# SamuelGong/FLASHE

Hardware: AMD Instinct MI355X
Metric: ciphertexts/sec (enc+agg+dec), 1e7-elem vector; achieved HBM GB/s fraction (higher is better)
Workload: dtype u128

## Files before the change

### flashe_amd/csrc/abi.hip

```cpp
#include "ctx.h"
#include "blockpool.h"

#include <algorithm>
#include <cstdarg>
#include <cstdio>
#include <cstdlib>
#include <cmath>
#include <cstring>
#include <mutex>
#include <new>
#include <string>
#include <vector>

using namespace flashe;

namespace {

struct AesTables {
    uint8_t sbox[256];
    uint32_t te0[256];
    AesTables()
    {
        uint8_t alog[256], lg[256];
        uint8_t x = 1;
// ... 761 lines not shown
        if (rc) return rc;
    }
    if (ctx->env.prf_backend != PRF_AUTO && ctx->env.prf_backend != PRF_TABLE) {
        for (int v = 0; v < n_vec; v++) {
            int rc = flashe_encrypt_dev(ctx, iter, idx[v], scheme, n, n_jobs, pt_dev[v], pt_limbs, ct_dev[v]);
            if (rc) return rc;
        }
        return FLASHE_OK;
    }
    return batch_shares(ctx, n_vec, [&](int v0, int nv) {
        return launch_prf_batch(ctx->env, iter, scheme == FLASHE_SCHEME_DOUBLE, nv, idx + v0, pt_dev + v0, pt_limbs, ct_dev + v0, n, n_jobs);
    });
}

static int check_range(flashe_ctx *ctx, uint64_t n, uint64_t first, uint64_t count);
static int check_u32(flashe_ctx *ctx, uint64_t n, uint32_t n_jobs)
{
    if (ctx->int_bits > 32) return fail(ctx, FLASHE_EINVAL, "the uint32 layout needs int_bits <= 32, this ctx has %d", ctx->int_bits);
    if (n >= (1ull << 32)) return fail(ctx, FLASHE_EINVAL, "the uint32 layout needs n < 2^32");
    if (n_jobs == 0) return fail(ctx, FLASHE_EINVAL, "n_jobs must be >= 1");
    if (ctx->env.prf_backend != PRF_AUTO && ctx->env.prf_backend != PRF_TABLE) return fail(ctx, FLASHE_EINVAL, "the uint32 layout runs on the table PRF only");
    if (!ctx->env.use_chain) return fail(ctx, FLASHE_EINVAL, "the uint32 layout needs the chained kernels (FLASHE_CHAIN=0 is set)");
    return FLASHE_OK;
}

int flashe_encrypt_batch_u32_dev(flashe_ctx *ctx, uint32_t iter, int scheme, uint64_t n, uint32_t n_jobs, int n_vec, const uint32_t *idx,
                                 const uint32_t *const *pt_dev, uint32_t *const *ct_dev)
{
    CHECK_CTX(ctx);
    if (int rc = check_scheme(ctx, scheme)) return rc;
// ... 21 lines not shown
    if (reinterpret_cast<uintptr_t>(sum_out_dev) & 3u) return fail(ctx, FLASHE_EINVAL, "sum_out_dev must be 4-byte aligned");
    if (n && ct_dev) { if (int rc = check_sum_apart(ctx, sum_out_dev, n_vec, pt_dev, ct_dev)) return rc; }
    if (scheme == FLASHE_SCHEME_DOUBLE && n && n_vec > 0 && n_vec <= kMaxUniformBatch && idx && pt_dev && ct_dev) {
        int rc = check_u32(ctx, n, n_jobs);
        if (rc || (rc = check_double_idx(ctx, scheme, idx, n_vec))) return rc;
        bool ok = true;
        for (int v = 0; v < n_vec && ok; v++)
            ok = pt_dev[v] && ct_dev[v] && !((reinterpret_cast<uintptr_t>(pt_dev[v]) | reinterpret_cast<uintptr_t>(ct_dev[v])) & 3u) && (v == 0 || idx[v] == idx[v - 1] + 1u);
        if (ok) {
            LaunchEnv env = ctx->env;
            env.elem32 = 1;
            std::vector<uint32_t> sidx(idx, idx + n_vec);
            sidx.push_back(idx[n_vec - 1] + 1u);
            PrfChain ch{sidx.data(), n_vec, false, 0, n, reinterpret_cast<const uint64_t *const *>(pt_dev), 1, reinterpret_cast<uint64_t *const *>(ct_dev)};
            ch.sum_out_dev = reinterpret_cast<uint64_t *>(sum_out_dev);
            const hipError_t e = launch_prf_chains(env, iter, 1, &ch, n, n_jobs);
            if (e == hipSuccess) return FLASHE_OK;
            if (e != hipErrorNotSupported) HIP_TRY(ctx, e);
        }
    }
    int rc = flashe_encrypt_batch_u32_dev(ctx, iter, scheme, n, n_jobs, n_vec, idx, pt_dev, ct_dev);
    if (rc || n == 0) return rc;
    if (n_vec == 0) { HIP_TRY(ctx, hipMemsetAsync(sum_out_dev, 0, n * 4, ctx->env.stream)); return FLASHE_OK; }
    return flashe_aggregate_elem_u32_dev(ctx, n_vec, ct_dev, n, sum_out_dev);
}

int flashe_aggregate_decrypt_u32_dev(flashe_ctx *ctx, uint32_t iter, const uint32_t *add_idx, int n_add, const uint32_t *minus_idx, int n_minus,
                                     uint64_t n, uint32_t n_jobs, uint64_t first, uint64_t count, int C, const uint32_t *const *cts_dev,
                                     void *agg_out_dev, void *out_dev, int out_elem_bytes)
{
    CHECK_CTX(ctx);
    if (C < 1 || C > kMaxOps || !cts_dev || (count && !out_dev)) return fail(ctx, FLASHE_EINVAL, "aggregate_decrypt_u32: bad arguments (C = %d, at most %d)", C, kMaxOps);
    if (out_elem_bytes != 4 && out_elem_bytes != 8) return fail(ctx, FLASHE_EINVAL, "out_elem_bytes must be 4 or 8");
    if (n_add != 1 || n_minus < 0 || n_minus > 1 || !add_idx || (n_minus && !minus_idx))
        return fail(ctx, FLASHE_EINVAL, "aggregate_decrypt_u32: one add and at most one minus prefix (widen the vectors for prefix lists)");
    int rc = check_u32(ctx, n, n_jobs);
    if (rc) return rc;
    rc = check_range(ctx, n, first, count);
    if (rc) return rc;
    if (count == 0) return FLASHE_OK;
    if ((rc = check_operands(ctx, C, cts_dev, 4))) return rc;
    const uintptr_t need = static_cast<uintptr_t>(out_elem_bytes - 1);
    if ((reinterpret_cast<uintptr_t>(out_dev) | reinterpret_cast<uintptr_t>(agg_out_dev)) & need) return fail(ctx, FLASHE_EINVAL, "outputs must be %d-byte aligned", out_elem_bytes);
    LaunchEnv env = ctx->env;
    env.elem32 = 1;
    if (C == 1 && !agg_out_dev && out_elem_bytes == 4 && n_minus == 1) {
        const uint32_t sidx[2] = {add_idx[0], minus_idx[0]};
        const uint64_t *in1 = reinterpret_cast<const uint64_t *>(cts_dev[0]);
        uint64_t *out1 = static_cast<uint64_t *>(out_dev);
        PrfChain ch{sidx, 1, false, first, count, &in1, 1, &out1};
        const hipError_t e = launch_prf_chains(env, iter, 1, &ch, n, n_jobs);
        if (e == hipSuccess) return FLASHE_OK;
        if (e != hipErrorNotSupported) HIP_TRY(ctx, e);
    }
    HIP_TRY(ctx, launch_small_reduce_decrypt(env, iter, add_idx[0], n_minus == 1, n_minus ? minus_idx[0] : 0u, n, n_jobs, first, count, C,
                                             reinterpret_cast<const uint64_t *const *>(cts_dev), static_cast<uint64_t *>(agg_out_dev),
                                             static_cast<uint64_t *>(out_dev), out_elem_bytes));
    return FLASHE_OK;
}

int flashe_aggregate_elem_u32_dev(flashe_ctx *ctx, int C, const uint32_t *const *cts_dev, uint64_t n, uint32_t *out_dev)
// ... 19 lines not shown
{
    CHECK_CTX(ctx);
    if (n && (!in_dev || !out_dev)) return fail(ctx, FLASHE_EINVAL, "widen_u32: null vector");
    HIP_TRY(ctx, launch_widen_u32(ctx->env, n, in_dev, out_dev));
    return FLASHE_OK;
}

int flashe_narrow_u32_dev(flashe_ctx *ctx, uint64_t n, const uint64_t *in_dev, uint32_t *out_dev)
{
    CHECK_CTX(ctx);
    if (n && (!in_dev || !out_dev)) return fail(ctx, FLASHE_EINVAL, "narrow_u32: null vector");
    HIP_TRY(ctx, launch_narrow_u32(ctx->env, n, in_dev, out_dev));
    return FLASHE_OK;
}

static uint64_t *chain_dmask_begin(flashe_ctx *ctx, uint64_t count)
{
    flashe_ctx::ChainDmask &s = ctx->chain_dmask;
    s.valid = false;
    if (!ctx->chain_dmask_on || ctx->capturing || ctx->limbs != 2 || count == 0) return nullptr;
    if (ensure(ctx, s.d, vec_bytes(ctx, count)) != FLASHE_OK) {
        (void)hipGetLastError();
        ctx->err.clear();
        return nullptr;
    }
    return static_cast<uint64_t *>(s.d.p);
}

static void chain_dmask_commit(flashe_ctx *ctx, uint32_t iter, const uint32_t *idx, int n_vec, uint64_t n, uint32_t n_jobs, uint64_t first,
                               uint64_t count)
{
    flashe_ctx::ChainDmask &s = ctx->chain_dmask;
    s.iter = iter; s.key_epoch = ctx->key_epoch; s.add_idx = idx[n_vec - 1] + 1u; s.minus_idx = idx[0];
    s.n = n; s.n_jobs = n_jobs; s.first = first; s.count = count;
    s.valid = true;
}

static const uint64_t *chain_dmask_match(const flashe_ctx *ctx, uint32_t iter, const uint32_t *add_idx, int n_add, const uint32_t *minus_idx,
                                         int n_minus, uint64_t n, uint32_t n_jobs, uint64_t first, uint64_t count)
{
    const flashe_ctx::ChainDmask &s = ctx->chain_dmask;
    if (!s.valid || ctx->capturing || n_add != 1 || n_minus != 1 || count == 0) return nullptr;
    if (add_idx[0] != s.add_idx || minus_idx[0] != s.minus_idx || iter != s.iter || ctx->key_epoch != s.key_epoch || n != s.n ||
        n_jobs != s.n_jobs)
        return nullptr;
    if (first < s.first || first - s.first > s.count || count > s.count - (first - s.first)) return nullptr;
    return static_cast<const uint64_t *>(s.d.p) + (first - s.first) * 2;
}

int flashe_encrypt_batch_sum_dev(flashe_ctx *ctx, uint32_t iter, int scheme, uint64_t n, uint32_t n_jobs, int n_vec, const uint32_t *idx,
                                 const uint64_t *const *pt_dev, int pt_limbs, uint64_t *const *ct_dev, uint64_t *sum_out_dev)
{
    CHECK_CTX(ctx);
    if (!sum_out_dev && n && n_vec) return fail(ctx, FLASHE_EINVAL, "flashe_encrypt_batch_sum_dev: null sum_out_dev");
    if (n_vec > 0) { if (int rc = check_double_idx(ctx, scheme, idx, n_vec)) return rc; }
    if (n && n_vec) {
        if (int rc = check_sum_aligned(ctx, sum_out_dev)) return rc;
        if (int rc = check_sum_apart(ctx, sum_out_dev, n_vec, pt_dev, ct_dev)) return rc;
    }
    if (scheme == FLASHE_SCHEME_DOUBLE && n && n_vec > 0 && idx && pt_dev && ct_dev) {
        bool ok = true;
        for (int v = 0; v < n_vec && ok; v++) ok = pt_dev[v] && ct_dev[v];
        if (ok) {
            for (int v = 0; v < n_vec; v++) {
                int rc = check_prf_args(ctx, 1, scheme, n_jobs, ct_dev[v], pt_dev[v], pt_limbs);
                if (rc) return rc;
            }
            uint64_t *const dmask = chain_dmask_begin(ctx, n);
            const hipError_t e = launch_prf_batch_sum(ctx->env, iter, n_vec, idx, pt_dev, pt_limbs, ct_dev, sum_out_dev, n, n_jobs, 0, n, dmask);
            if (e == hipSuccess) {
                if (dmask) chain_dmask_commit(ctx, iter, idx, n_vec, n, n_jobs, 0, n);
                return FLASHE_OK;
            }
            if (e != hipErrorNotSupported) HIP_TRY(ctx, e);
        }
    }
    int rc = flashe_encrypt_batch_dev(ctx, iter, scheme, n, n_jobs, n_vec, idx, pt_dev, pt_limbs, ct_dev);
    if (rc || n == 0) return rc;
    if (n_vec == 0) { HIP_TRY(ctx, hipMemsetAsync(sum_out_dev, 0, n * ctx->limbs * 8, ctx->env.stream)); return FLASHE_OK; }
    return flashe_aggregate_elem_dev(ctx, n_vec, ct_dev, n, sum_out_dev);
}

int flashe_prf_jobs_dev(flashe_ctx *ctx, uint32_t iter, uint64_t n, uint32_t n_jobs, int n_entries, const flashe_prf_job *entries)
{
    CHECK_CTX(ctx);
    if (n_entries < 0 || (n_entries && !entries)) return fail(ctx, FLASHE_EINVAL, "bad job list");
// ... 813 lines not shown
    int rc = check_range(ctx, n, first, count);
    if (rc || (rc = check_double_idx(ctx, scheme, idx, n_vec))) return rc;
    if (n_jobs == 0) return fail(ctx, FLASHE_EINVAL, "n_jobs must be >= 1");
    if (ctx->env.prf_backend != PRF_AUTO && ctx->env.prf_backend != PRF_TABLE) return fail(ctx, FLASHE_EINVAL, "encrypt_batch_range runs on the table PRF only");
    for (int v = 0; v < n_vec; v++) {
        if (count && (!pt_dev[v] || !ct_dev[v])) return fail(ctx, FLASHE_EINVAL, "null vector %d", v);
        if (sum_out_dev && (ct_dev[v] == sum_out_dev || pt_dev[v] == sum_out_dev))
            return fail(ctx, FLASHE_EINVAL, "sum_out_dev must not be one of the plaintext or ciphertext vectors");
        rc = check_prf_args(ctx, 1, scheme, n_jobs, ct_dev[v], pt_dev[v], pt_limbs);
        if (rc) return rc;
    }
    if (sum_out_dev && (rc = check_sum_aligned(ctx, sum_out_dev))) return rc;
    if (count == 0) return FLASHE_OK;
    if (n_vec == 0) { if (sum_out_dev) HIP_TRY(ctx, hipMemsetAsync(sum_out_dev, 0, vec_bytes(ctx, count), ctx->env.stream)); return FLASHE_OK; }
    if (sum_out_dev && scheme == FLASHE_SCHEME_DOUBLE) {
        uint64_t *const dmask = chain_dmask_begin(ctx, count);
        const hipError_t e = launch_prf_batch_sum(ctx->env, iter, n_vec, idx, pt_dev, pt_limbs, ct_dev, sum_out_dev, n, n_jobs, first, count, dmask);
        if (e == hipSuccess) {
            if (dmask) chain_dmask_commit(ctx, iter, idx, n_vec, n, n_jobs, first, count);
            return FLASHE_OK;
        }
        if (e != hipErrorNotSupported) HIP_TRY(ctx, e);
    }
    rc = batch_shares(ctx, n_vec, [&](int v0, int nv) {
        return launch_prf_batch_range(ctx->env, iter, scheme == FLASHE_SCHEME_DOUBLE, nv, idx + v0, pt_dev + v0, pt_limbs, ct_dev + v0, n, n_jobs,
                                      first, count);
    });
    if (rc) return rc;
    if (sum_out_dev) return flashe_aggregate_elem_dev(ctx, n_vec, ct_dev, count, sum_out_dev);
    return FLASHE_OK;
}

int flashe_decrypt_range_dev(flashe_ctx *ctx, uint32_t iter, const uint32_t *add_idx, int n_add, const uint32_t *minus_idx,
                             int n_minus, uint64_t n, uint32_t n_jobs, uint64_t first, uint64_t count,
                             const uint64_t *in_dev, uint64_t *out_dev)
{
    CHECK_CTX(ctx);
    if (count && (!in_dev || !out_dev)) return fail(ctx, FLASHE_EINVAL, "null vector");
    int rc = check_prf_args(ctx, n_add, n_minus, n_jobs, out_dev, in_dev, ctx->limbs);
    if (rc || (rc = check_range(ctx, n, first, count))) return rc;
    if (n_add == 0 && n_minus == 0) {
        HIP_TRY(ctx, launch_combine(ctx->env, count, in_dev, ctx->limbs, nullptr, nullptr, out_dev));
        return FLASHE_OK;
    }
    if (const uint64_t *d = chain_dmask_match(ctx, iter, add_idx, n_add, minus_idx, n_minus, n, n_jobs, first, count)) {
        HIP_TRY(ctx, launch_combine(ctx->env, count, in_dev, ctx->limbs, d, nullptr, out_dev));
        return FLASHE_OK;
    }
    HIP_TRY(ctx, prf_lists(ctx, iter, add_idx, n_add, minus_idx, n_minus, n, n_jobs, first, count, in_dev, ctx->limbs, out_dev));
    return FLASHE_OK;
}

int flashe_combine_dev(flashe_ctx *ctx, uint64_t n, const uint64_t *in_dev, int in_limbs, const uint64_t *add_dev,
                       const uint64_t *minus_dev, uint64_t *out_dev)
{
    CHECK_CTX(ctx);
    if (n && (!in_dev || !out_dev)) return fail(ctx, FLASHE_EINVAL, "null vector");
    if (in_limbs != 1 && in_limbs != ctx->limbs) return fail(ctx, FLASHE_EINVAL, "in_limbs must be 1 or %d", ctx->limbs);
    if (ctx->limbs == 2 && (!aligned16(out_dev) || !aligned16(add_dev) || !aligned16(minus_dev) || (in_limbs == 2 && !aligned16(in_dev))))
        return fail(ctx, FLASHE_EINVAL, "device vectors must be 16-byte aligned");
    HIP_TRY(ctx, launch_combine(ctx->env, n, in_dev, in_limbs, add_dev, minus_dev, out_dev));
// ... 1312 lines not shown
```

### flashe_amd/csrc/ctx.h

```cpp
#pragma once
#include "flashe.h"
#include "kernels.h"
#include "blockpool.h"

#include <string>
#include <vector>

struct flashe_ctx {
    int device = 0;
    int device_cus = 0;
    int int_bits = 0;
    int limbs = 0;
    bool own_stream = false;
    flashe::LaunchEnv env{};
    uint32_t *te0_dev = nullptr;
    uint32_t *rkw_dev = nullptr;
    uint32_t *rkp_dev = nullptr;
    std::string err;
    struct Buf { void *p = nullptr; size_t cap = 0; };
    Buf summaries;
    Buf stream_tmp;
    Buf acc_tmp[2];
    Buf sp_ws;
    Buf bounds;
    Buf mt_ws;
    Buf codec_tab;
    Buf tensor_ws;
    Buf tensor_tab;
    Buf stat_ws;
    hipEvent_t ev_foreign = nullptr;
    struct Prepared { Buf add, minus; uint64_t n = 0; bool valid = false, has_minus = false; uint32_t iter = 0, add_idx = 0, minus_idx = 0; };
    Prepared prep_enc, prep_dec;
    struct ChainDmask { Buf d; uint64_t n = 0, first = 0, count = 0; uint32_t iter = 0, key_epoch = 0, add_idx = 0, minus_idx = 0, n_jobs = 0; bool valid = false; };
    ChainDmask chain_dmask;
    bool chain_dmask_on = true;
    flashe_pool::StagingPool *staging = nullptr;
    bool capturing = false;
    uint32_t key_epoch = 0;
    hipEvent_t ev_copy[2] = {nullptr, nullptr};
    uint32_t *err_flag_host = nullptr;
};

namespace flashe_host {

int fail(flashe_ctx *ctx, int code, const char *fmt, ...) __attribute__((format(printf, 3, 4)));

inline size_t vec_bytes(const flashe_ctx *ctx, uint64_t n) { return static_cast<size_t>(n) * ctx->limbs * 8; }

// ... 36 lines not shown
```

### flashe_amd/csrc/kernels.h

```cpp
#pragma once
#include <hip/hip_runtime.h>
#include <stdint.h>

namespace flashe {

struct RoundKeys { uint32_t w[60]; };

struct CodecLayer {
    uint64_t start;
    const void *x;
    double p0, p1, p2;
    int x_is_f64, pad_;
};
struct Codec {
    const void *x;
    const double *u;
    double alpha, scale, den;
    int x_is_f64, n_layers;
    double *fout;
    double ac, two_a, uden;
    const CodecLayer *layers;
    uint64_t k0;
};

// ... 67 lines not shown
hipError_t launch_prf_jobs(const LaunchEnv &env, uint32_t iter, bool dbl, int n_entries, const PrfJob *jobs, uint64_t n,
                           uint32_t n_jobs);

struct PrfChain {
    const uint32_t *idx;
    int n_out;
    bool single;
    uint64_t first, count;
    const uint64_t *const *in_dev;
    int in_limbs;
    uint64_t *const *out_dev;
    uint64_t *sum_out_dev = nullptr;
    uint64_t *dmask_dev = nullptr;
};
hipError_t launch_prf_chains(const LaunchEnv &env, uint32_t iter, int n_chains, const PrfChain *chains, uint64_t n, uint32_t n_jobs);

hipError_t launch_combine(const LaunchEnv &env, uint64_t n, const uint64_t *in_dev, int in_limbs,
                          const uint64_t *add_dev, const uint64_t *minus_dev, uint64_t *out_dev);

hipError_t launch_combine_batch(const LaunchEnv &env, uint64_t n, int n_vec, const uint64_t *const *in_dev, int in_limbs,
                                const uint64_t *const *add_dev, const uint64_t *const *minus_dev, uint64_t *const *out_dev);
hipError_t launch_combine_batch_sum(const LaunchEnv &env, uint64_t n, int n_vec, const uint64_t *const *in_dev, int in_limbs,
                                    const uint64_t *const *add_dev, const uint64_t *const *minus_dev, uint64_t *const *out_dev, uint64_t *sum_out_dev,
                                    const uint64_t *dec_add_dev = nullptr, const uint64_t *dec_minus_dev = nullptr, uint64_t *dec_out_dev = nullptr);

constexpr int kMaxOps = 64;
struct PtrTable { const uint64_t *p[kMaxOps]; };

hipError_t launch_small_reduce_decrypt(const LaunchEnv &env, uint32_t iter, uint32_t add_idx, bool has_minus, uint32_t minus_idx, uint64_t n,
                                       uint32_t n_jobs, uint64_t first, uint64_t count, int C, const uint64_t *const *ops, uint64_t *agg_out_dev,
                                       uint64_t *out_dev, int out_elem_bytes = 8);
// ... 162 lines not shown
```

### flashe_amd/csrc/kernels.hip

```cpp
#include "device_common.h"
#include <type_traits>

namespace flashe {

struct IdxLists {
    uint32_t add[kMaxIdx];
    uint32_t minus[kMaxIdx];
};

struct PrfParams {
    const uint64_t *in;
    uint64_t *out;
    const uint32_t *te0;
    uint64_t n;
    uint64_t first, count;
    uint64_t blk_first, blk_count;
    uint64_t mask_lo, mask_hi;
    uint32_t iter;
    int in_limbs;
    int n_add, n_minus;
    uint32_t n_jobs;
    int b, m;
    Codec cq;
};
// ... 988 lines not shown
#pragma unroll
    for (; t + 4 <= M; t += 4) {
        u32x4_a4 x;
        x[0] = r[t] & mask; x[1] = r[t + 1] & mask; x[2] = r[t + 2] & mask; x[3] = r[t + 3] & mask;
        *reinterpret_cast<u32x4_a4 *>(q + t) = x;
    }
    if (M - t >= 2) {
        u32x2_a4 x;
        x[0] = r[t] & mask; x[1] = r[t + 1] & mask;
        *reinterpret_cast<u32x2_a4 *>(q + t) = x;
        t += 2;
    }
    if (t < M) q[t] = r[t] & mask;
}

template <int B, bool SINGLE, class SRC = void, class OT = uint32_t>
__device__ __forceinline__ void small_chain_fast32(const RoundKeys &rk, const LaneRegs lr, const uint32_t *pre_lds, int sbase, int n_streams,
                                                   const uint64_t *const *in_tab, uint64_t *const *out_tab, const CtrVar &xA, const CtrVar &xB,
                                                   uint64_t kA, uint64_t kB, uint32_t *sum32, bool prio,
                                                   const uint32_t *__restrict__ te4, bool uni, uint32_t x3A, uint32_t x3B, const SRC *src = nullptr)
{
    constexpr int M = 128 / B;
    constexpr uint32_t mask = B >= 32 ? 0xffffffffu : ((1u << (B & 31)) - 1u);
    uint32_t psA[M], psB[M], accA[M], accB[M];
#pragma unroll
    for (int t = 0; t < M; t++) { psA[t] = 0u; psB[t] = 0u; accA[t] = 0u; accB[t] = 0u; }
    auto prefix_of = [&](const uint4 &v) {
        return CtrPrefix{{static_cast<uint32_t>(__builtin_amdgcn_readfirstlane(v.x)), static_cast<uint32_t>(__builtin_amdgcn_readfirstlane(v.y)),
                          static_cast<uint32_t>(__builtin_amdgcn_readfirstlane(v.z)), static_cast<uint32_t>(__builtin_amdgcn_readfirstlane(v.w))}};
    };
    uint4 pv = *reinterpret_cast<const uint4 *>(pre_lds + 4 * sbase);
    auto emit = [&](int link, const u128 SA, const u128 SB, const DirectPt<M> &dA, const DirectPt<M> &dB) {
        uint32_t csA[M], csB[M];
#pragma unroll
        for (int t = 0; t < M; t++) {
            csA[t] = static_cast<uint32_t>(SA >> (B * t));
            csB[t] = static_cast<uint32_t>(SB >> (B * t));
        }
// ... 26 lines not shown
                dA = src->template block<M>(link, kA, 0);
                dB = src->template block<M>(link, kB, 1);
            }
        }
        uint32_t s[2][4];
        if (uni) {
            const CtrUniform UA = ctr_uniform(rk, te4, pre, x3A), UB = ctr_uniform(rk, te4, pre, x3B);
            ctr_round2(lr, pre.u[0], xA.v[0], UA, s[0]);
            ctr_round2(lr, pre.u[0], xB.v[0], UB, s[1]);
            aes256_rounds<2, 3>(rk, lr, s, prio);
        } else {
            ctr_round1(pre, xA, s[0]);
            ctr_round1(pre, xB, s[1]);
            aes256_rounds<2, 2>(rk, lr, s, prio);
        }
        emit(link, words_to_u128(s[0]), words_to_u128(s[1]), dA, dB);
    }
    if (sum32) {
        direct32_put<M>(sum32 + kA, accA, mask);
        direct32_put<M>(sum32 + kB, accB, mask);
    }
}

__device__ __forceinline__ u128 slot_diff(u128 prev, u128 cur, u128 top, int b)
{
    if (b == 64) {
        const uint64_t lo = static_cast<uint64_t>(prev) - static_cast<uint64_t>(cur), hi = static_cast<uint64_t>(prev >> 64) - static_cast<uint64_t>(cur >> 64);
        return (static_cast<u128>(hi) << 64) | lo;
    }
    return ((prev | top) - (cur & ~top)) ^ ((prev ^ ~cur) & top);
}

template <bool PAIR, class ET = uint64_t, int B = 0>
__global__ __launch_bounds__(kSmallThreads) void prf_small_chain_kernel(const RoundKeys rk, const SmallChainTable tb, int n_chains, const SmallParams p)
{
    constexpr bool COHORT = false;
    const CohortCodec cc{};
#include "prf_small_chain_body.inc"
}

template <int B>
__global__ __launch_bounds__(kSmallThreads) void prf_small_cohort_kernel(const RoundKeys rk, const SmallChainTable tb, int n_chains, const SmallParams p,
                                                                          const CohortCodec cc)
{
    constexpr bool PAIR = true, COHORT = true;
    using ET = uint32_t;
#include "prf_small_chain_body.inc"
}

struct SparseCohortTail {
    const double *zzz;
    uint64_t *zeros;
    const double *u_n;
    uint64_t u_stride, n;
    double alpha, scale, den;
    int f64, n_clients;
};
template <int B>
__global__ __launch_bounds__(kSmallThreads) void prf_small_sparse_cohort_kernel(const RoundKeys rk, const SmallChainTable tb, int n_chains, const SmallParams p,
                                                                                 const CohortCodec cc, const SparseCohortTail tail)
{
    constexpr bool PAIR = true, COHORT = true;
    using ET = uint64_t;
    if (blockIdx.x == 0 && threadIdx.x < static_cast<unsigned>(tail.n_clients)) {
        const int c = threadIdx.x;
        const double v = tail.zzz[c], u = tail.u_n[static_cast<uint64_t>(c) * tail.u_stride];
        const uint64_t q = tail.f64 ? quantize_one<double>(v, tail.alpha, tail.scale, tail.den, u)
                                    : quantize_one<float>(static_cast<float>(v), static_cast<float>(tail.alpha), static_cast<float>(tail.scale),
                                                          static_cast<float>(tail.den), u);
        tail.zeros[c] = q;
        tb.out[c][tail.n] = q;
    }
#include "prf_small_chain_body.inc"
}


template <int CB, int EPL>
// ... 882 lines not shown
    case 2: case 3: SRD_LAUNCH(2); break;
    case 4: case 5: case 6: case 7: SRD_LAUNCH(4); break;
    default: SRD_LAUNCH(8); break;
    }
#undef SRD_LAUNCH
    return hipGetLastError();
}

static int small_swp_prio(const LaunchEnv &env, const SmallParams &p, int longest)
{
    int prio = env.elem32 ? (!p.no_fixed_width && fixed32_width(env.b) && (env.b != 20 || longest <= 1)) : (p.m <= 4 && !p.no_direct);
    { static const int v = FLASHE_TUNE_ENV("FLASHE_SMALL_PRIO") ? atoi(FLASHE_TUNE_ENV("FLASHE_SMALL_PRIO")) : -1; if (v >= 0) prio = v; }
    return prio;
}

static hipError_t launch_small_chains(const LaunchEnv &env, uint32_t iter, int n_chains, const PrfChain *chains, uint64_t n, uint32_t n_jobs)
{
    if (env.codec || n >= (1ull << 32) || n == 0) return hipErrorNotSupported;
    SmallParams p = small_params_of(env, iter, n, n_jobs);
    bool summed = false;
    for (int i = 0; i < n_chains; i++) summed |= chains[i].sum_out_dev != nullptr;
    if (summed && !(env.elem32 && !p.no_fixed_width && fixed32_width(env.b) && n_chains == 1 && !chains[0].single &&
                    chains[0].n_out <= kMaxLinks))
        return hipErrorNotSupported;
    if (env.elem32) {
        if (env.b > 32) return hipErrorInvalidValue;
        p.no_direct = 1;
    }
    int longest = 0;
    for (int i = 0; i < n_chains; i++) longest = std::max(longest, chains[i].n_out);
    p.swp_prio = small_swp_prio(env, p, longest);
    struct Piece { const PrfChain *ch; int l0, l1; uint64_t blk_first, blk_count; };
    std::vector<Piece> pieces;
    uint64_t total_blocks = 0;
    for (int i = 0; i < n_chains; i++) {
        const PrfChain &c = chains[i];
        if (c.count == 0 || c.n_out == 0) continue;
        if (c.in_dev && c.in_limbs != 1) return hipErrorInvalidValue;
        const uint64_t bf = block_of(c.first, n, n_jobs, p.m), bc = block_of(c.first + c.count - 1, n, n_jobs, p.m) - bf + 1;
// ... 37 lines not shown
            for (int l = 0; l < len; l++) {
                tb.in[links + l] = c.in_dev ? c.in_dev[pc.l0 + l] : nullptr;
                tb.out[links + l] = c.out_dev[pc.l0 + l];
            }
            tb.sum_out[nc] = c.sum_out_dev;
            const uint64_t t = (pc.blk_count + tile - 1) / tile;
            wend += t * static_cast<uint64_t>(ns);
            tb.wend[nc] = wend;
            tiles += t;
            links += len; streams += ns; nc++;
        }
        const uint64_t cus = static_cast<uint64_t>(env.num_cus);
        const int grid = static_cast<int>(tiles < cus ? tiles : cus);
        if (env.elem32) {
            const int fixed = (pair && !p.no_fixed_width) ? env.b : 0;
            switch (fixed) {
#define FLASHE_FIXED32(B) case B: hipLaunchKernelGGL((prf_small_chain_kernel<true, uint32_t, B>), dim3(grid), dim3(kSmallThreads), 0, env.stream, env.rk, tb, nc, p); break;
                FLASHE_FIXED32_WIDTHS(FLASHE_FIXED32)
#undef FLASHE_FIXED32
            default:
                if (pair) hipLaunchKernelGGL((prf_small_chain_kernel<true, uint32_t>), dim3(grid), dim3(kSmallThreads), 0, env.stream, env.rk, tb, nc, p);
                else hipLaunchKernelGGL((prf_small_chain_kernel<false, uint32_t>), dim3(grid), dim3(kSmallThreads), 0, env.stream, env.rk, tb, nc, p);
            }
        } else if (pair && env.b == 64 && !p.no_fixed_width && !p.no_direct)
            hipLaunchKernelGGL((prf_small_chain_kernel<true, uint64_t, 64>), dim3(grid), dim3(kSmallThreads), 0, env.stream, env.rk, tb, nc, p);
        else if (pair) hipLaunchKernelGGL((prf_small_chain_kernel<true>), dim3(grid), dim3(kSmallThreads), 0, env.stream, env.rk, tb, nc, p);
        else hipLaunchKernelGGL((prf_small_chain_kernel<false>), dim3(grid), dim3(kSmallThreads), 0, env.stream, env.rk, tb, nc, p);
        const hipError_t e = hipGetLastError();
        if (e != hipSuccess) return e;
    }
    return hipSuccess;
}

bool small_cohort_admits(const LaunchEnv &env, int n_vec, uint64_t n, uint32_t n_jobs, bool summed)
{
    if (!env.use_chain || env.b > 32 || !fixed32_width(env.b) || env.codec || !table_prf(env) || n_vec < 1 || n_vec > kMaxLinks) return false;
    if (n == 0 || n >= (1ull << 32) || n_jobs == 0 || small_no_fixed_width()) return false;
    return !summed || block_of(n - 1, n, n_jobs, 128 / env.b) + 1 >= 2 * 128 * static_cast<uint64_t>(env.num_cus) * (kSmallThreads / 64);
}

static SmallParams small_cohort_params(const LaunchEnv &env, uint32_t iter, int n_vec, uint64_t n, uint32_t n_jobs, uint64_t *blocks)
{
    LaunchEnv e32 = env;
    e32.elem32 = 1;
    SmallParams p = small_params_of(e32, iter, n, n_jobs);
    p.no_direct = 1;
// ... 208 lines not shown
```

### flashe_amd/csrc/prf_small_chain_body.inc

```
    static_assert(!COHORT || (PAIR && B != 0 && B <= 32), "the cohort front end rides on the paired chain at a compile-time width");
    (void)cc;
    constexpr bool LIMB_OUT = COHORT && sizeof(ET) == 8;
    static_assert(B == 0 || (PAIR && ((sizeof(ET) == 4 && B <= 32) || (sizeof(ET) == 8 && (B == 64 || LIMB_OUT)))), "compile-time widths: the paired kernel, compact layout or int_bits 64");
    constexpr uint32_t WAVES = kSmallThreads / 64, TILE = PAIR ? 128u : 64u;
    constexpr int MB = B ? 128 / B : 1;
    __shared__ uint32_t tab[kTabWords];
    __shared__ uint32_t scratch[(kSmallThreads / 64) * 256 + 8];
    __shared__ __attribute__((aligned(16))) uint32_t pre_lds[(kMaxLinks + kMaxChains) * 4];
    __shared__ uint64_t d_tlo[kMaxChains], d_cend[kMaxChains];
    const uint32_t iter = p.iter + p.te0[kIterShiftWord];
    fill_tables(tab, p.te0);
    const LaneRegs lr = lane_regs(tab);
    {
        const int last = n_chains - 1;
        const int n_streams = tb.sbase[last] + tb.len[last] + ((tb.flags[last] & 1) ? 0 : 1);
        for (int s = threadIdx.x; s < n_streams; s += kSmallThreads) {
            const CtrPrefix c = ctr_prefix(rk, lr, iter, tb.idx[s], 0u);
            *reinterpret_cast<uint4 *>(pre_lds + 4 * s) = make_uint4(c.u[0], c.u[1], c.u[2], c.u[3]);
        }
        if (threadIdx.x < static_cast<unsigned>(n_chains)) {
            const int i = threadIdx.x;
            const uint64_t Wt = tb.wend[last], cw = i ? tb.wend[i - 1] : 0;
            const uint32_t w = tb.len[i] + ((tb.flags[i] & 1) ? 0u : 1u);
            uint64_t a, b, T;
// ... 84 lines not shown
                constexpr int kU2MaxStreams = 2;
                const uint32_t bA = static_cast<uint32_t>(__builtin_amdgcn_readfirstlane(ctrA)), bB = static_cast<uint32_t>(__builtin_amdgcn_readfirstlane(ctrB));
                const bool uni = n_streams <= kU2MaxStreams && __ballot(ctrA - bA == lane && ctrB - bB == lane) == ~0ull &&
                                 (bA & 255u) <= 192u && (bB & 255u) <= 192u;
                if constexpr (LIMB_OUT) {
                    const CohortDirect csrc{cc, tb.in + link0, link0, {layA, layB}};
                    small_chain_fast32<B, true, CohortDirect, uint64_t>(rk, lr, pre_lds, sbase, n_streams, tb.in + link0, tb.out + link0, xA, xB, j0A - first, j0B - first,
                                                                        nullptr, p.swp_prio != 0, p.te0, uni, bA ^ rk.w[3], bB ^ rk.w[3], &csrc);
                    continue;
                } else if constexpr (COHORT) {
                    const CohortDirect csrc{cc, tb.in + link0, link0, {layA, layB}};
                    small_chain_fast32<B, false>(rk, lr, pre_lds, sbase, n_streams, tb.in + link0, tb.out + link0, xA, xB, j0A - first, j0B - first, sum32, p.swp_prio != 0,
                                                 p.te0, uni, bA ^ rk.w[3], bB ^ rk.w[3], &csrc);
                    continue;
                }
                if (single) small_chain_fast32<B, true>(rk, lr, pre_lds, sbase, n_streams, tb.in + link0, tb.out + link0, xA, xB, j0A - first, j0B - first, sum32, p.swp_prio != 0,
                                                        p.te0, uni, bA ^ rk.w[3], bB ^ rk.w[3]);
                else small_chain_fast32<B, false>(rk, lr, pre_lds, sbase, n_streams, tb.in + link0, tb.out + link0, xA, xB, j0A - first, j0B - first, sum32, p.swp_prio != 0,
                                                  p.te0, uni, bA ^ rk.w[3], bB ^ rk.w[3]);
                continue;
            }
        }
        if (PAIR) {
            for (int c = 0; c < n_streams; c++) {
                const CtrPrefix pre = load_prefix(pre_lds, sbase + c);
                const int link = single ? c : c - 1;
                WalkPt ptA{}, ptB{};
                DirectPt<MB> dA{}, dB{};
                u64x2 qA = {0ull, 0ull}, qB = {0ull, 0ull};
                if (B == 64) {
// ... 62 lines not shown
                        if (fastA) small_walk32(row0, lane, e0A, DA, ptA, ein, eout, first, p, wblk0, wo0);
                        else small_walk(row0, lane, vA, cntA, j0A, DA, ein, eout, first, range_end, p);
                        if (fastB) small_walk32(row0, lane, e0B, DB, ptB, ein, eout, first, p, wblk0, wo0);
                        else small_walk(row0, lane, vB, cntB, j0B, DB, ein, eout, first, range_end, p);
                    }
                }
                prevA = SA; prevB = SB;
            }
            if constexpr (B != 0 && B != 64) {
                if (sum32) {
                    constexpr uint32_t bmask = B >= 32 ? 0xffffffffu : ((1u << (B & 31)) - 1u);
                    if (fastA) direct32_put<MB>(sum32 + (j0A - first), accA, bmask);
                    if (fastB) direct32_put<MB>(sum32 + (j0B - first), accB, bmask);
                }
            }
        } else {
            for (int c = 0; c < n_streams; c += 2) {
                const bool has1 = c + 1 < n_streams;
                const CtrPrefix pre0 = load_prefix(pre_lds, sbase + c), pre1 = load_prefix(pre_lds, sbase + (has1 ? c + 1 : c));
                const int l0 = single ? c : c - 1;
                WalkPt pt0{}, pt1{};
                if (fastA && l0 >= 0) pt0 = small_walk32_load(reinterpret_cast<const ET *>(tb.in[link0 + l0]), e0A, first, lane, m32);
                if (fastA && has1) pt1 = small_walk32_load(reinterpret_cast<const ET *>(tb.in[link0 + l0 + 1]), e0A, first, lane, m32);
                uint32_t s[2][4];
                ctr_round1(pre0, xA, s[0]);
                ctr_round1(pre1, xA, s[1]);
                aes256_rounds<2, 2>(rk, lr, s, true);
                const u128 S0 = words_to_u128(s[0]), S1 = words_to_u128(s[1]);
                if (l0 >= 0) {
                    const u128 D = single ? S0 : slot_diff(prevA, S0, top, p.b);
// ... 19 lines not shown
```

### flashe_amd/csrc/stream.hip

```cpp
#include "device_common.h"

namespace flashe {

__global__ __launch_bounds__(kStreamThreads) void widen_u32_kernel(uint64_t n, const uint32_t *in, uint64_t *out)
{
    for (uint64_t j = static_cast<uint64_t>(blockIdx.x) * kStreamThreads + threadIdx.x; j < n; j += static_cast<uint64_t>(gridDim.x) * kStreamThreads)
        out[j] = in[j];
}
__global__ __launch_bounds__(kStreamThreads) void narrow_u32_kernel(uint64_t n, const uint64_t *in, uint32_t *out)
{
    for (uint64_t j = static_cast<uint64_t>(blockIdx.x) * kStreamThreads + threadIdx.x; j < n; j += static_cast<uint64_t>(gridDim.x) * kStreamThreads)
        out[j] = static_cast<uint32_t>(in[j]);
}
hipError_t launch_widen_u32(const LaunchEnv &env, uint64_t n, const uint32_t *in_dev, uint64_t *out_dev)
{
    if (n == 0) return hipSuccess;
    hipLaunchKernelGGL(widen_u32_kernel, dim3(stream_grid(env, n)), dim3(kStreamThreads), 0, env.stream, n, in_dev, out_dev);
    return hipGetLastError();
}
hipError_t launch_narrow_u32(const LaunchEnv &env, uint64_t n, const uint64_t *in_dev, uint32_t *out_dev)
{
    if (n == 0) return hipSuccess;
    hipLaunchKernelGGL(narrow_u32_kernel, dim3(stream_grid(env, n)), dim3(kStreamThreads), 0, env.stream, n, in_dev, out_dev);
    return hipGetLastError();
// ... 11 lines not shown
        if (minus) v -= ld128_nt(minus + 2 * j);
        st128_nt(out + 2 * j, v & mask);
    }
}

__global__ __launch_bounds__(kStreamThreads) void combine_small_kernel(uint64_t n, const uint64_t *in, const uint64_t *add,
                                                                       const uint64_t *minus, uint64_t *out, uint64_t mask)
{
    for (uint64_t j = static_cast<uint64_t>(blockIdx.x) * kStreamThreads + threadIdx.x; j < n;
         j += static_cast<uint64_t>(gridDim.x) * kStreamThreads) {
        uint64_t v = in[j];
        if (add) v += add[j];
        if (minus) v -= minus[j];
        out[j] = v & mask;
    }
}

constexpr int kMaxCombine = 64;
struct CombineTable {
    const uint64_t *in[kMaxCombine], *add[kMaxCombine], *minus[kMaxCombine];
    uint64_t *out[kMaxCombine];
};

template <bool WIDE>
__global__ __launch_bounds__(kStreamThreads) void combine_batch_kernel(uint64_t n, const CombineTable tb, int in_limbs, uint64_t mask_lo, uint64_t mask_hi)
{
    const int v = blockIdx.y;
    const uint64_t *in = tb.in[v], *add = tb.add[v], *minus = tb.minus[v];
    uint64_t *out = tb.out[v];
    const u128 mask = (static_cast<u128>(mask_hi) << 64) | mask_lo;
// ... 1542 lines not shown
```

Measured before the change: 72.71 billion.

## Emit u32 decrypt mask from summed encrypt chain and reuse in decrypt

```diff
diff --git a/flashe_amd/csrc/abi.hip b/flashe_amd/csrc/abi.hip
--- a/flashe_amd/csrc/abi.hip
+++ b/flashe_amd/csrc/abi.hip
@@ -799,6 +799,11 @@
 }
 
 static int check_range(flashe_ctx *ctx, uint64_t n, uint64_t first, uint64_t count);
+static uint64_t *chain_dmask_begin(flashe_ctx *ctx, uint64_t count, int elem_bytes);
+static void chain_dmask_commit(flashe_ctx *ctx, uint32_t iter, const uint32_t *idx, int n_vec, uint64_t n, uint32_t n_jobs, uint64_t first,
+                               uint64_t count, int elem_bytes);
+static const void *chain_dmask_match(const flashe_ctx *ctx, uint32_t iter, const uint32_t *add_idx, int n_add, const uint32_t *minus_idx,
+                                     int n_minus, uint64_t n, uint32_t n_jobs, uint64_t first, uint64_t count, int elem_bytes);
 static int check_u32(flashe_ctx *ctx, uint64_t n, uint32_t n_jobs)
 {
     if (ctx->int_bits > 32) return fail(ctx, FLASHE_EINVAL, "the uint32 layout needs int_bits <= 32, this ctx has %d", ctx->int_bits);
@@ -850,11 +855,23 @@
             sidx.push_back(idx[n_vec - 1] + 1u);
             PrfChain ch{sidx.data(), n_vec, false, 0, n, reinterpret_cast<const uint64_t *const *>(pt_dev), 1, reinterpret_cast<uint64_t *const *>(ct_dev)};
             ch.sum_out_dev = reinterpret_cast<uint64_t *>(sum_out_dev);
-            const hipError_t e = launch_prf_chains(env, iter, 1, &ch, n, n_jobs);
+            hipError_t e = hipErrorNotSupported;
+            ctx->chain_dmask.valid = false;
+            if (uint64_t *const dmask = small_dmask_admits(env, n_vec, n, n_jobs) ? chain_dmask_begin(ctx, n, 4) : nullptr) {
+                ch.dmask_dev = dmask;
+                e = launch_prf_chains(env, iter, 1, &ch, n, n_jobs);
+                if (e == hipSuccess) {
+                    chain_dmask_commit(ctx, iter, idx, n_vec, n, n_jobs, 0, n, 4);
+                    return FLASHE_OK;
+                }
+                ch.dmask_dev = nullptr;
+            }
+            if (e == hipErrorNotSupported) e = launch_prf_chains(env, iter, 1, &ch, n, n_jobs);
             if (e == hipSuccess) return FLASHE_OK;
             if (e != hipErrorNotSupported) HIP_TRY(ctx, e);
         }
     }
+    ctx->chain_dmask.valid = false;
     int rc = flashe_encrypt_batch_u32_dev(ctx, iter, scheme, n, n_jobs, n_vec, idx, pt_dev, ct_dev);
     if (rc || n == 0) return rc;
     if (n_vec == 0) { HIP_TRY(ctx, hipMemsetAsync(sum_out_dev, 0, n * 4, ctx->env.stream)); return FLASHE_OK; }
@@ -881,6 +898,10 @@
     LaunchEnv env = ctx->env;
     env.elem32 = 1;
     if (C == 1 && !agg_out_dev && out_elem_bytes == 4 && n_minus == 1) {
+        if (const void *d = chain_dmask_match(ctx, iter, add_idx, n_add, minus_idx, n_minus, n, n_jobs, first, count, 4)) {
+            HIP_TRY(ctx, launch_combine_u32(env, count, cts_dev[0], static_cast<const uint32_t *>(d), static_cast<uint32_t *>(out_dev)));
+            return FLASHE_OK;
+        }
         const uint32_t sidx[2] = {add_idx[0], minus_idx[0]};
         const uint64_t *in1 = reinterpret_cast<const uint64_t *>(cts_dev[0]);
         uint64_t *out1 = static_cast<uint64_t *>(out_dev);
@@ -930,12 +951,13 @@
     return FLASHE_OK;
 }
 
-static uint64_t *chain_dmask_begin(flashe_ctx *ctx, uint64_t count)
+static uint64_t *chain_dmask_begin(flashe_ctx *ctx, uint64_t count, int elem_bytes)
 {
     flashe_ctx::ChainDmask &s = ctx->chain_dmask;
     s.valid = false;
-    if (!ctx->chain_dmask_on || ctx->capturing || ctx->limbs != 2 || count == 0) return nullptr;
-    if (ensure(ctx, s.d, vec_bytes(ctx, count)) != FLASHE_OK) {
+    if (!ctx->chain_dmask_on || ctx->capturing || count == 0) return nullptr;
+    if (elem_bytes == 16 ? ctx->limbs != 2 : (elem_bytes != 4 || ctx->int_bits > 32)) return nullptr;
+    if (ensure(ctx, s.d, static_cast<size_t>(count) * elem_bytes) != FLASHE_OK) {
         (void)hipGetLastError();
         ctx->err.clear();
         return nullptr;
@@ -944,24 +966,25 @@
 }
 
 static void chain_dmask_commit(flashe_ctx *ctx, uint32_t iter, const uint32_t *idx, int n_vec, uint64_t n, uint32_t n_jobs, uint64_t first,
-                               uint64_t count)
+                               uint64_t count, int elem_bytes)
 {
     flashe_ctx::ChainDmask &s = ctx->chain_dmask;
+    s.elem_bytes = elem_bytes;
     s.iter = iter; s.key_epoch = ctx->key_epoch; s.add_idx = idx[n_vec - 1] + 1u; s.minus_idx = idx[0];
     s.n = n; s.n_jobs = n_jobs; s.first = first; s.count = count;
     s.valid = true;
 }
 
-static const uint64_t *chain_dmask_match(const flashe_ctx *ctx, uint32_t iter, const uint32_t *add_idx, int n_add, const uint32_t *minus_idx,
-                                         int n_minus, uint64_t n, uint32_t n_jobs, uint64_t first, uint64_t count)
+static const void *chain_dmask_match(const flashe_ctx *ctx, uint32_t iter, const uint32_t *add_idx, int n_add, const uint32_t *minus_idx,
+                                     int n_minus, uint64_t n, uint32_t n_jobs, uint64_t first, uint64_t count, int elem_bytes)
 {
     const flashe_ctx::ChainDmask &s = ctx->chain_dmask;
-    if (!s.valid || ctx->capturing || n_add != 1 || n_minus != 1 || count == 0) return nullptr;
+    if (!s.valid || s.elem_bytes != elem_bytes || ctx->capturing || n_add != 1 || n_minus != 1 || count == 0) return nullptr;
     if (add_idx[0] != s.add_idx || minus_idx[0] != s.minus_idx || iter != s.iter || ctx->key_epoch != s.key_epoch || n != s.n ||
         n_jobs != s.n_jobs)
         return nullptr;
     if (first < s.first || first - s.first > s.count || count > s.count - (first - s.first)) return nullptr;
-    return static_cast<const uint64_t *>(s.d.p) + (first - s.first) * 2;
+    return static_cast<const char *>(s.d.p) + (first - s.first) * static_cast<uint64_t>(elem_bytes);
 }
 
 int flashe_encrypt_batch_sum_dev(flashe_ctx *ctx, uint32_t iter, int scheme, uint64_t n, uint32_t n_jobs, int n_vec, const uint32_t *idx,
@@ -982,10 +1005,10 @@
                 int rc = check_prf_args(ctx, 1, scheme, n_jobs, ct_dev[v], pt_dev[v], pt_limbs);
                 if (rc) return rc;
             }
-            uint64_t *const dmask = chain_dmask_begin(ctx, n);
+            uint64_t *const dmask = chain_dmask_begin(ctx, n, 16);
             const hipError_t e = launch_prf_batch_sum(ctx->env, iter, n_vec, idx, pt_dev, pt_limbs, ct_dev, sum_out_dev, n, n_jobs, 0, n, dmask);
             if (e == hipSuccess) {
-                if (dmask) chain_dmask_commit(ctx, iter, idx, n_vec, n, n_jobs, 0, n);
+                if (dmask) chain_dmask_commit(ctx, iter, idx, n_vec, n, n_jobs, 0, n, 16);
                 return FLASHE_OK;
             }
             if (e != hipErrorNotSupported) HIP_TRY(ctx, e);
@@ -1829,10 +1852,10 @@
     if (count == 0) return FLASHE_OK;
     if (n_vec == 0) { if (sum_out_dev) HIP_TRY(ctx, hipMemsetAsync(sum_out_dev, 0, vec_bytes(ctx, count), ctx->env.stream)); return FLASHE_OK; }
     if (sum_out_dev && scheme == FLASHE_SCHEME_DOUBLE) {
-        uint64_t *const dmask = chain_dmask_begin(ctx, count);
+        uint64_t *const dmask = chain_dmask_begin(ctx, count, 16);
         const hipError_t e = launch_prf_batch_sum(ctx->env, iter, n_vec, idx, pt_dev, pt_limbs, ct_dev, sum_out_dev, n, n_jobs, first, count, dmask);
         if (e == hipSuccess) {
-            if (dmask) chain_dmask_commit(ctx, iter, idx, n_vec, n, n_jobs, first, count);
+            if (dmask) chain_dmask_commit(ctx, iter, idx, n_vec, n, n_jobs, first, count, 16);
             return FLASHE_OK;
         }
         if (e != hipErrorNotSupported) HIP_TRY(ctx, e);
@@ -1858,8 +1881,8 @@
         HIP_TRY(ctx, launch_combine(ctx->env, count, in_dev, ctx->limbs, nullptr, nullptr, out_dev));
         return FLASHE_OK;
     }
-    if (const uint64_t *d = chain_dmask_match(ctx, iter, add_idx, n_add, minus_idx, n_minus, n, n_jobs, first, count)) {
-        HIP_TRY(ctx, launch_combine(ctx->env, count, in_dev, ctx->limbs, d, nullptr, out_dev));
+    if (const void *d = chain_dmask_match(ctx, iter, add_idx, n_add, minus_idx, n_minus, n, n_jobs, first, count, 16)) {
+        HIP_TRY(ctx, launch_combine(ctx->env, count, in_dev, ctx->limbs, static_cast<const uint64_t *>(d), nullptr, out_dev));
         return FLASHE_OK;
     }
     HIP_TRY(ctx, prf_lists(ctx, iter, add_idx, n_add, minus_idx, n_minus, n, n_jobs, first, count, in_dev, ctx->limbs, out_dev));
diff --git a/flashe_amd/csrc/ctx.h b/flashe_amd/csrc/ctx.h
--- a/flashe_amd/csrc/ctx.h
+++ b/flashe_amd/csrc/ctx.h
@@ -31,7 +31,7 @@
     hipEvent_t ev_foreign = nullptr;
     struct Prepared { Buf add, minus; uint64_t n = 0; bool valid = false, has_minus = false; uint32_t iter = 0, add_idx = 0, minus_idx = 0; };
     Prepared prep_enc, prep_dec;
-    struct ChainDmask { Buf d; uint64_t n = 0, first = 0, count = 0; uint32_t iter = 0, key_epoch = 0, add_idx = 0, minus_idx = 0, n_jobs = 0; bool valid = false; };
+    struct ChainDmask { Buf d; uint64_t n = 0, first = 0, count = 0; uint32_t iter = 0, key_epoch = 0, add_idx = 0, minus_idx = 0, n_jobs = 0; int elem_bytes = 0; bool valid = false; };
     ChainDmask chain_dmask;
     bool chain_dmask_on = true;
     flashe_pool::StagingPool *staging = nullptr;
diff --git a/flashe_amd/csrc/kernels.h b/flashe_amd/csrc/kernels.h
--- a/flashe_amd/csrc/kernels.h
+++ b/flashe_amd/csrc/kernels.h
@@ -105,7 +105,9 @@
     uint64_t *dmask_dev = nullptr;
 };
 hipError_t launch_prf_chains(const LaunchEnv &env, uint32_t iter, int n_chains, const PrfChain *chains, uint64_t n, uint32_t n_jobs);
-
+bool small_dmask_admits(const LaunchEnv &env, int n_vec, uint64_t n, uint32_t n_jobs);
+
+hipError_t launch_combine_u32(const LaunchEnv &env, uint64_t n, const uint32_t *in_dev, const uint32_t *d_dev, uint32_t *out_dev);
 hipError_t launch_combine(const LaunchEnv &env, uint64_t n, const uint64_t *in_dev, int in_limbs,
                           const uint64_t *add_dev, const uint64_t *minus_dev, uint64_t *out_dev);
 
diff --git a/flashe_amd/csrc/kernels.hip b/flashe_amd/csrc/kernels.hip
--- a/flashe_amd/csrc/kernels.hip
+++ b/flashe_amd/csrc/kernels.hip
@@ -1026,14 +1026,17 @@
     if (t < M) q[t] = r[t] & mask;
 }
 
-template <int B, bool SINGLE, class SRC = void, class OT = uint32_t>
+template <int B, bool SINGLE, class SRC = void, class OT = uint32_t, int DM = 0>
 __device__ __forceinline__ void small_chain_fast32(const RoundKeys &rk, const LaneRegs lr, const uint32_t *pre_lds, int sbase, int n_streams,
                                                    const uint64_t *const *in_tab, uint64_t *const *out_tab, const CtrVar &xA, const CtrVar &xB,
                                                    uint64_t kA, uint64_t kB, uint32_t *sum32, bool prio,
-                                                   const uint32_t *__restrict__ te4, bool uni, uint32_t x3A, uint32_t x3B, const SRC *src = nullptr)
+                                                   const uint32_t *__restrict__ te4, bool uni, uint32_t x3A, uint32_t x3B, const SRC *src = nullptr,
+                                                   uint32_t *dm32 = nullptr)
 {
     constexpr int M = 128 / B;
     constexpr uint32_t mask = B >= 32 ? 0xffffffffu : ((1u << (B & 31)) - 1u);
+    static_assert(DM == 0 || (!SINGLE && sizeof(OT) == 4 && M >= 4), "the decrypt mask: double-mask compact chains, a block's mask words hold its raw first stream");
+    u128 f0A = 0, f0B = 0;
     uint32_t psA[M], psB[M], accA[M], accB[M];
 #pragma unroll
     for (int t = 0; t < M; t++) { psA[t] = 0u; psB[t] = 0u; accA[t] = 0u; accB[t] = 0u; }
@@ -1090,12 +1093,42 @@
             ctr_round1(pre, xB, s[1]);
             aes256_rounds<2, 2>(rk, lr, s, prio);
         }
+        if constexpr (DM != 0) {
+            if (c == 0) {
+                if constexpr (DM == 1) {
+                    f0A = words_to_u128(s[0]); f0B = words_to_u128(s[1]);
+                } else {
+                    u32x4_a4 a, b;
+                    a[0] = s[0][0]; a[1] = s[0][1]; a[2] = s[0][2]; a[3] = s[0][3];
+                    b[0] = s[1][0]; b[1] = s[1][1]; b[2] = s[1][2]; b[3] = s[1][3];
+                    *reinterpret_cast<u32x4_a4 *>(dm32 + kA) = a;
+                    *reinterpret_cast<u32x4_a4 *>(dm32 + kB) = b;
+                }
+            }
+        }
         emit(link, words_to_u128(s[0]), words_to_u128(s[1]), dA, dB);
     }
     if (sum32) {
         direct32_put<M>(sum32 + kA, accA, mask);
         direct32_put<M>(sum32 + kB, accB, mask);
     }
+    if constexpr (DM != 0) {
+        if constexpr (DM == 2) {
+            const uint32_t *qa = dm32 + kA, *qb = dm32 + kB;
+            asm volatile("" : "+v"(qa), "+v"(qb));
+            const u32x4_a4 a = *reinterpret_cast<const u32x4_a4 *>(qa), b = *reinterpret_cast<const u32x4_a4 *>(qb);
+            uint32_t wa[4] = {a[0], a[1], a[2], a[3]}, wb[4] = {b[0], b[1], b[2], b[3]};
+            f0A = words_to_u128(wa); f0B = words_to_u128(wb);
+        }
+        uint32_t mA[M], mB[M];
+#pragma unroll
+        for (int t = 0; t < M; t++) {
+            mA[t] = psA[t] - static_cast<uint32_t>(f0A >> (B * t));
+            mB[t] = psB[t] - static_cast<uint32_t>(f0B >> (B * t));
+        }
+        direct32_put<M>(dm32 + kA, mA, mask);
+        direct32_put<M>(dm32 + kB, mB, mask);
+    }
 }
 
 __device__ __forceinline__ u128 slot_diff(u128 prev, u128 cur, u128 top, int b)
@@ -1111,6 +1144,23 @@
 __global__ __launch_bounds__(kSmallThreads) void prf_small_chain_kernel(const RoundKeys rk, const SmallChainTable tb, int n_chains, const SmallParams p)
 {
     constexpr bool COHORT = false;
+    constexpr int DMASK = 0;
+    uint32_t *const dmask = nullptr;
+    const CohortCodec cc{};
+#include "prf_small_chain_body.inc"
+}
+
+#ifndef FLASHE_SMALL_DMASK_FORM
+#define FLASHE_SMALL_DMASK_FORM(B) ((B) == 16 ? 2 : 1)
+#endif
+template <int B> constexpr int kSmallDmaskForm = FLASHE_SMALL_DMASK_FORM(B);
+template <int B>
+__global__ __launch_bounds__(kSmallThreads) void prf_small_chain_dmask_kernel(const RoundKeys rk, const SmallChainTable tb, int n_chains, const SmallParams p,
+                                                                               uint32_t *__restrict__ dmask)
+{
+    constexpr bool PAIR = true, COHORT = false;
+    constexpr int DMASK = kSmallDmaskForm<B>;
+    using ET = uint32_t;
     const CohortCodec cc{};
 #include "prf_small_chain_body.inc"
 }
@@ -1120,6 +1170,8 @@
                                                                           const CohortCodec cc)
 {
     constexpr bool PAIR = true, COHORT = true;
+    constexpr int DMASK = 0;
+    uint32_t *const dmask = nullptr;
     using ET = uint32_t;
 #include "prf_small_chain_body.inc"
 }
@@ -1137,6 +1189,8 @@
                                                                                  const CohortCodec cc, const SparseCohortTail tail)
 {
     constexpr bool PAIR = true, COHORT = true;
+    constexpr int DMASK = 0;
+    uint32_t *const dmask = nullptr;
     using ET = uint64_t;
     if (blockIdx.x == 0 && threadIdx.x < static_cast<unsigned>(tail.n_clients)) {
         const int c = threadIdx.x;
@@ -2049,6 +2103,11 @@
     return prio;
 }
 
+static bool small_dmask_width(int b)
+{
+    return fixed32_width(b);
+}
+
 static hipError_t launch_small_chains(const LaunchEnv &env, uint32_t iter, int n_chains, const PrfChain *chains, uint64_t n, uint32_t n_jobs)
 {
     if (env.codec || n >= (1ull << 32) || n == 0) return hipErrorNotSupported;
@@ -2058,6 +2117,12 @@
     if (summed && !(env.elem32 && !p.no_fixed_width && fixed32_width(env.b) && n_chains == 1 && !chains[0].single &&
                     chains[0].n_out <= kMaxLinks))
         return hipErrorNotSupported;
+    uint32_t *dmask = nullptr;
+    for (int i = 0; i < n_chains; i++) {
+        if (!chains[i].dmask_dev) continue;
+        if (!chains[i].sum_out_dev || !small_dmask_width(env.b) || chains[i].count == 0) return hipErrorNotSupported;
+        dmask = reinterpret_cast<uint32_t *>(chains[i].dmask_dev);
+    }
     if (env.elem32) {
         if (env.b > 32) return hipErrorInvalidValue;
         p.no_direct = 1;
@@ -2125,6 +2190,14 @@
         const int grid = static_cast<int>(tiles < cus ? tiles : cus);
         if (env.elem32) {
             const int fixed = (pair && !p.no_fixed_width) ? env.b : 0;
+            if (dmask) {
+                switch (fixed) {
+#define FLASHE_FIXED32(B) case B: hipLaunchKernelGGL((prf_small_chain_dmask_kernel<B>), dim3(grid), dim3(kSmallThreads), 0, env.stream, env.rk, tb, nc, p, dmask); break;
+                    FLASHE_FIXED32_WIDTHS(FLASHE_FIXED32)
+#undef FLASHE_FIXED32
+                default: return hipErrorNotSupported;
+                }
+            } else
             switch (fixed) {
 #define FLASHE_FIXED32(B) case B: hipLaunchKernelGGL((prf_small_chain_kernel<true, uint32_t, B>), dim3(grid), dim3(kSmallThreads), 0, env.stream, env.rk, tb, nc, p); break;
                 FLASHE_FIXED32_WIDTHS(FLASHE_FIXED32)
@@ -2141,6 +2214,11 @@
         if (e != hipSuccess) return e;
     }
     return hipSuccess;
+}
+
+bool small_dmask_admits(const LaunchEnv &env, int n_vec, uint64_t n, uint32_t n_jobs)
+{
+    return small_dmask_width(env.b) && small_cohort_admits(env, n_vec, n, n_jobs, true);
 }
 
 bool small_cohort_admits(const LaunchEnv &env, int n_vec, uint64_t n, uint32_t n_jobs, bool summed)
diff --git a/flashe_amd/csrc/prf_small_chain_body.inc b/flashe_amd/csrc/prf_small_chain_body.inc
--- a/flashe_amd/csrc/prf_small_chain_body.inc
+++ b/flashe_amd/csrc/prf_small_chain_body.inc
@@ -1,5 +1,7 @@
     static_assert(!COHORT || (PAIR && B != 0 && B <= 32), "the cohort front end rides on the paired chain at a compile-time width");
     (void)cc;
+    (void)dmask;
+    static_assert(DMASK == 0 || (PAIR && !COHORT && B != 0 && B <= 32 && sizeof(ET) == 4), "the decrypt mask rides on the summed compact chain at a compile-time width");
     constexpr bool LIMB_OUT = COHORT && sizeof(ET) == 8;
     static_assert(B == 0 || (PAIR && ((sizeof(ET) == 4 && B <= 32) || (sizeof(ET) == 8 && (B == 64 || LIMB_OUT)))), "compile-time widths: the paired kernel, compact layout or int_bits 64");
     constexpr uint32_t WAVES = kSmallThreads / 64, TILE = PAIR ? 128u : 64u;
@@ -122,6 +124,11 @@
                                                  p.te0, uni, bA ^ rk.w[3], bB ^ rk.w[3], &csrc);
                     continue;
                 }
+                if constexpr (DMASK != 0) {
+                    small_chain_fast32<B, false, void, uint32_t, DMASK>(rk, lr, pre_lds, sbase, n_streams, tb.in + link0, tb.out + link0, xA, xB, j0A - first, j0B - first,
+                                                                        sum32, p.swp_prio != 0, p.te0, uni, bA ^ rk.w[3], bB ^ rk.w[3], nullptr, dmask);
+                    continue;
+                }
                 if (single) small_chain_fast32<B, true>(rk, lr, pre_lds, sbase, n_streams, tb.in + link0, tb.out + link0, xA, xB, j0A - first, j0B - first, sum32, p.swp_prio != 0,
                                                         p.te0, uni, bA ^ rk.w[3], bB ^ rk.w[3]);
                 else small_chain_fast32<B, false>(rk, lr, pre_lds, sbase, n_streams, tb.in + link0, tb.out + link0, xA, xB, j0A - first, j0B - first, sum32, p.swp_prio != 0,
@@ -214,6 +221,22 @@
                     if (fastB) direct32_put<MB>(sum32 + (j0B - first), accB, bmask);
                 }
             }
+            if constexpr (DMASK != 0) {
+                const CtrPrefix pre = load_prefix(pre_lds, sbase);
+                uint32_t s[2][4];
+                ctr_round1(pre, xA, s[0]);
+                ctr_round1(pre, xB, s[1]);
+                aes256_rounds<2, 2>(rk, lr, s, p.swp_prio != 0);
+                const u128 FA = words_to_u128(s[0]), FB = words_to_u128(s[1]);
+                const DirectPt<MB> zero{};
+                uint32_t unused[MB];
+#pragma unroll
+                for (int t = 0; t < MB; t++) unused[t] = 0u;
+                if (fastA) direct32_store<B, uint32_t>(dmask, j0A - first, zero, prevA, FA, false, unused);
+                else small_walk(row0, lane, vA, cntA, j0A, slot_diff(prevA, FA, top, p.b), static_cast<const ET *>(nullptr), reinterpret_cast<ET *>(dmask), first, range_end, p);
+                if (fastB) direct32_store<B, uint32_t>(dmask, j0B - first, zero, prevB, FB, false, unused);
+                else small_walk(row0, lane, vB, cntB, j0B, slot_diff(prevB, FB, top, p.b), static_cast<const ET *>(nullptr), reinterpret_cast<ET *>(dmask), first, range_end, p);
+            }
         } else {
             for (int c = 0; c < n_streams; c += 2) {
                 const bool has1 = c + 1 < n_streams;
diff --git a/flashe_amd/csrc/stream.hip b/flashe_amd/csrc/stream.hip
--- a/flashe_amd/csrc/stream.hip
+++ b/flashe_amd/csrc/stream.hip
@@ -49,6 +49,34 @@
         if (minus) v -= minus[j];
         out[j] = v & mask;
     }
+}
+
+typedef uint32_t u32x4_a4 __attribute__((ext_vector_type(4), aligned(4)));
+__global__ __launch_bounds__(kStreamThreads) void combine_u32_kernel(uint64_t n, const uint32_t *in, const uint32_t *__restrict__ d, uint32_t *out,
+                                                                     uint32_t mask)
+{
+    uint64_t head = ((16u - (reinterpret_cast<uintptr_t>(out) & 15u)) & 15u) / 4u;
+    if (head > n) head = n;
+    const uint64_t quads = (n - head) / 4u, tail0 = head + 4u * quads;
+    const uint64_t tid = static_cast<uint64_t>(blockIdx.x) * kStreamThreads + threadIdx.x;
+    if (tid < head) out[tid] = (in[tid] + d[tid]) & mask;
+    else if (tid - head < n - tail0) out[tail0 + (tid - head)] = (in[tail0 + (tid - head)] + d[tail0 + (tid - head)]) & mask;
+    for (uint64_t q = tid; q < quads; q += static_cast<uint64_t>(gridDim.x) * kStreamThreads) {
+        const uint64_t k = head + 4u * q;
+        const u32x4_a4 a = __builtin_nontemporal_load(reinterpret_cast<const u32x4_a4 *>(in + k));
+        const u32x4_a4 b = __builtin_nontemporal_load(reinterpret_cast<const u32x4_a4 *>(d + k));
+        u32x4_a4 r;
+        r[0] = (a[0] + b[0]) & mask; r[1] = (a[1] + b[1]) & mask; r[2] = (a[2] + b[2]) & mask; r[3] = (a[3] + b[3]) & mask;
+        __builtin_nontemporal_store(r, reinterpret_cast<u32x4_a4 *>(out + k));
+    }
+}
+hipError_t launch_combine_u32(const LaunchEnv &env, uint64_t n, const uint32_t *in_dev, const uint32_t *d_dev, uint32_t *out_dev)
+{
+    if (n == 0) return hipSuccess;
+    if (env.b > 32) return hipErrorInvalidValue;
+    const uint32_t mask = env.b >= 32 ? 0xffffffffu : ((1u << env.b) - 1u);
+    hipLaunchKernelGGL(combine_u32_kernel, dim3(stream_grid(env, n / 4 + 8)), dim3(kStreamThreads), 0, env.stream, n, in_dev, d_dev, out_dev, mask);
+    return hipGetLastError();
 }
 
 constexpr int kMaxCombine = 64;
```

Result: no change. 72.80 billion (median of 3 runs) (+0.1%).
